# Exidekat/TransformerUpscaler

Measured on AMD Instinct MI355X. Metric: images/sec, FastTransformer 2x 720p->1080p inference, higher is better.
Workload: dtype bf16

## Files before the change

include/tupscale_hip.h:

```cpp
#ifndef TUPSCALE_HIP_H
#define TUPSCALE_HIP_H

#ifdef __cplusplus
extern "C" {
#endif

int tup_abi_version(void);

int tup_conv3x3_c3_fwd(const float* x, const void* wp, const float* bias, const float* in_mask,
                       const void* out_mask, void* out, int B, int H, int W, int relu, void* stream);

int tup_conv3x3_c64_fwd(const void* x, const void* wp, const float* bias, const void* add,
                        const void* mask, void* out, int B, int H, int W, int ntiles, int r,
                        int cout_valid, int relu, int out_mode, int in_r, void* stream);

int tup_decoder_fused_fwd(const void* x, const void* w1, const float* b1, const void* wz, const float* b2,
                          float* seamv, float* cseam, float* out, int B, int H, int W, void* stream);

int tup_conv1_compact_fwd(const float* x, void* xc, int B, int H, int W, void* stream);
int tup_conv12_fused_fwd(const void* xc, const void* w1, const float* b1, const void* w2, const float* b2, void* out,
                         int B, int H, int W, void* stream);

int tup_conv5x5_c64_planar_fwd(const void* x, const void* wp, const float* bias, const void* wv,
                               const float* bv, float* out, int B, int H, int W, int r, int relu, void* stream);

int tup_conv3x3_planar_fwd(const float* x, const float* w28, const float* bias, const float* add,
                           float* out, int B, int H, int W, int r, int clamp01, void* stream);

int tup_resize_aa_fwd(const float* in, float* out, const int* ymin, const int* ysize, const float* yw,
                      int KY, const int* xmin, const int* xsize, const float* xw, int KX, int planes,
                      int Hi, int Wi, int Ho, int Wo, int clamp01, void* stream);

int tup_tail_stream_r2_fwd(const float* x, const float* wfu_t, const float* bfu, const float* wfc_t, const float* bfc,
                           const float* ui, float* out, int B, int H, int W, int clamp01, void* stream);

int tup_tail_stream_r2_resize_fwd(const float* x, const float* wfu_t, const float* bfu, const float* wfc_t, const float* bfc,
                                  const float* ui, float* out, const int* ymin, const int* ysize, const float* yw, int KY,
                                  const int* xmin, const int* xsize, const float* xw, int KX, const int* oxb, const int* oyb,
                                  int B, int H, int W, int Ho, int Wo, int sc, int band_h, int ext, int clamp01, void* stream);

int tup_tail_fused_fwd(const float* x, const float* wfu, const float* bfu, const float* wfc, const float* bfc,
                       const float* ui, float* out, const int* ymin, const int* ysize, const float* yw, int KY,
                       const int* xmin, const int* xsize, const float* xw, int KX, int B, int H, int W, int r,
                       int Ho, int Wo, int EH, int EW, int clamp01, void* stream);

int tup_clamp01_fwd(const float* in, float* out, long long n, void* stream);

int tup_layernorm_fwd(const float* x, const float* gamma, const float* beta, void* y,
                      float* mean, float* rstd, int M, void* stream);

int tup_relpos_bias_expand(const float* table, float* frag, void* stream);

int tup_window_attn_fwd(const void* qkv, const float* bias_frag, void* out, float* lse, int nwin, float drop_p,
                        unsigned int drop_seed, void* stream);

int tup_gemm_tokens_fwd(const void* A, int a_dtype, int lda, const void* Wt, const float* bias,
                        const float* res, const void* aux, void* out, int ldo, int M, int N, int K,
                        int epilogue, float drop_p, unsigned int drop_seed, void* stream);

int tup_ln_gemm_fwd(const float* x, const float* gamma, const float* beta, const void* Wt,
                    const float* bias, void* out, int M, int N, void* stream);

// ... 206 lines not shown
```

transformerupscaler_amd/_lib.py:

```python
from __future__ import annotations

import ctypes
import os
from ctypes import c_double, c_float, c_int, c_longlong, c_uint, c_void_p

_HERE = os.path.dirname(os.path.abspath(__file__))
LIB_PATH = os.environ.get("TUP_LIB_PATH") or os.path.join(_HERE, "libtupscale_hip.so")
ABI_VERSION = 15

P = c_void_p
I = c_int
F = c_float
U = c_uint

SIGNATURES = {
    "tup_abi_version": [],
    "tup_conv3x3_c3_fwd": [P, P, P, P, P, P, I, I, I, I, P],
    "tup_conv3x3_c64_fwd": [P, P, P, P, P, P, I, I, I, I, I, I, I, I, I, P],
    "tup_conv5x5_c64_planar_fwd": [P, P, P, P, P, P, I, I, I, I, I, P],
    "tup_decoder_fused_fwd": [P, P, P, P, P, P, P, P, I, I, I, P],
    "tup_conv1_compact_fwd": [P, P, I, I, I, P],
    "tup_conv12_fused_fwd": [P, P, P, P, P, P, I, I, I, P],
    "tup_conv3x3_planar_fwd": [P, P, P, P, P, I, I, I, I, I, P],
    "tup_resize_aa_fwd": [P, P, P, P, P, I, P, P, P, I, I, I, I, I, I, I, P],
    "tup_tail_fused_fwd": [P, P, P, P, P, P, P, P, P, P, I, P, P, P, I, I, I, I, I, I, I, I, I, I, P],
    "tup_tail_stream_r2_fwd": [P, P, P, P, P, P, P, I, I, I, I, P],
    "tup_tail_stream_r2_resize_fwd": [P] * 7 + [P, P, P, I, P, P, P, I, P, P] + [I] * 9 + [P],
    "tup_clamp01_fwd": [P, P, c_longlong, P],
    "tup_layernorm_fwd": [P, P, P, P, P, P, I, P],
    "tup_relpos_bias_expand": [P, P, P],
    "tup_window_attn_fwd": [P, P, P, P, I, F, U, P],
    "tup_gemm_tokens_fwd": [P, I, I, P, P, P, P, P, I, I, I, I, I, F, U, P],
    "tup_ln_gemm_fwd": [P, P, P, P, P, P, I, I, P],
    "tup_fused_mlp_fwd": [P, P, P, P, P, P, P, I, P],
    "tup_patch_embed_fwd": [P, P, P, P, I, I, I, P],
    "tup_patch_unembed_fwd": [P, I, P, P, P, P, I, I, I, P],
    "tup_rt_patch_embed_fwd": [P, P, P, P, P, I, I, I, P],
    "tup_rt_patch_unembed_fwd": [P, P, P, P, P, I, I, I, P],
    "tup_rt_attention_fwd": [P, P, P, I, I, F, U, P],
    "tup_rt_attention_bwd": [P, P, P, P, P, P, I, I, F, U, P],
    "tup_layernorm128_fwd": [P, P, P, P, P, P, I, P],
    "tup_layernorm128_bwd": [P, P, P, P, P, P, P, P, P, I, P, F, U, P],
    "tup_rt_patch_wgrad": [P, P, P, I, I, I, P],
    "tup_conv3x3_c64_wgrad_s2d": [P, P, P, P, I, I, I, I, I, P],
    "tup_rt_bicubic_bwd": [P] * 10 + [I, I, I, I, I, P],
    "tup_rt_bicubic_bwd_banded": [P] * 7 + [I, P, P, I, P, P, I, I, I, I, I, P, P],
    "tup_relpos_bias_expand_h": [P, P, I, P],
    "tup_relpos_bias_expand_n_h": [P, P, I, P],
    "tup_window_attn_bwd_h": [P, P, P, P, P, P, P, P, I, I, F, U, P],
    "tup_relpos_bias_reduce_h": [P, P, I, P],
# ... 116 lines not shown
```

transformerupscaler_amd/csrc/check_resources.py:

```python
#!/usr/bin/env python3
import json
import os
import re
import subprocess
import sys

GUARDED = [
    ("fused_attn.hip", ["fused_qkv_attn_kernel"]),
    ("block_stream.hip", ["blocks_stream_kernel"]),
    ("fused_blocks.hip", ["fused_mlp_v2_kernel"]),
    ("conv3x3_c64.hip", ["conv_c64_persistent_kernel", "bra_rows_persistent_kernel", "conv3_thin_rows_kernel"]),
    ("conv_thin.hip", ["conv3x3_c3_persistent_kernel"]),
    ("decoder_fused.hip", ["decoder_fused_kernel"]),
    ("conv12_fused.hip", ["conv12_fused_kernel"]),
    ("gemm_tokens.hip", ["gemm_panel2_kernel", "patch_embed_kernel"]),
    ("conv_bwd.hip", ["conv3x3_wgrad_c64_kernel", "conv3x3_wgrad_thin_kernel", "conv3x3_wgrad_c64_det_kernel", "conv3x3_wgrad_thin_det_kernel"]),
    ("branch_a_train.hip", ["bra_wgrad_kernel"]),
    ("gemm_wgrad.hip", ["gemm_wgrad_wide_kernel"]),
    ("gemm_wgrad.hip", ["gemm_wgrad_kernelILi0ELi0ELb1E", "gemm_wgrad_kernelILi0ELi1ELb1E", "gemm_wgrad_kernelILi1ELi0ELb1E",
                        "gemm_wgrad_kernelILi1ELi1ELb1E", "gemm_wgrad_kernelILi1ELi2ELb1E", "colsum_kernelILb0ELb1E", "colsum_kernelILb1ELb1E"]),
    ("attention_bwd.hip", ["layernorm_bwd_kernelILi2ELb1E", "layernorm_bwd_kernelILi3ELb1E"]),
    ("quality_loss.hip", ["quality_loss_bwd_kernel"]),
    ("grad_accumulate.hip", ["grad_accumulate_kernel"]),
    ("step_guard.hip", ["grad_sumsq_kernel", "guard_finish_kernel", "adam_guarded_kernel"]),
    ("patch_pairs.hip", ["patch_pairs_kernel"]),
]
EXEMPT = re.compile(r"fused_qkv_attn_kernel<true, true, true>|fused_qkv_attn_kernelILb1ELb1ELb1E|fused_mlp_v2_kernelILi[1-9]|blocks_stream_kernel<true>|blocks_stream_kernelILb1E")
ALLOWED_BYTES = {"fused_mlp_v2_kernelILi0E": 72}

FIELDS = {
    "sgprs": r"TotalSGPRs: (\d+)", "vgprs": r" VGPRs: (\d+)", "agprs": r"AGPRs: (\d+)",
    "scratch_bytes_per_lane": r"ScratchSize \[bytes/lane\]: (\d+)", "waves_per_simd": r"Occupancy \[waves/SIMD\]: (\d+)",
    "sgpr_spill": r"SGPRs Spill: (\d+)", "vgpr_spill": r"VGPRs Spill: (\d+)",
}


def demangle(names):
    try:
        out = subprocess.run(["c++filt"], input="\n".join(names), capture_output=True, text=True, check=True).stdout.split("\n")
        return dict(zip(names, out))
    except Exception:
        return {n: n for n in names}


def parse(path):
    txt = open(path, errors="replace").read()
    parts = re.split(r"remark: Function Name: (\S+)", txt)
    recs = {}
# ... 58 lines not shown
```

transformerupscaler_amd/csrc/decoder_fused.hip:

```cpp
#include "common.h"

namespace {

constexpr int TH = 8, TW = 32, HALO_W = TW + 2, HALO_H = TH + 2, NPIX_HALO = HALO_H * HALO_W;
constexpr int IN_BYTES = NPIX_HALO * 128, IN_CHUNKS = NPIX_HALO * 8;
constexpr int WROWS = 64, WSLAB = WROWS * 128, WCHUNKS = 9 * WROWS * 8;
constexpr size_t DEC_LDS = (size_t)9 * WSLAB + 2 * (size_t)IN_BYTES + 256;
static_assert(DEC_LDS <= 163840, "LDS budget");

__device__ __attribute__((aligned(16))) unsigned int dec_zero_line[4] = {0u, 0u, 0u, 0u};

#define TUP_ADD_DPP(a, v, ctrl) asm("v_add_f32_dpp %0, %1, %0 " ctrl " row_mask:0xf bank_mask:0xf bound_ctrl:1" : "+v"(a) : "v"(v))

__global__ __launch_bounds__(512, 2) void decoder_fused_kernel(
    const bf16_t* __restrict__ x, const bf16_t* __restrict__ wp, const float* __restrict__ bias,
    const bf16_t* __restrict__ wz, float* __restrict__ part, float* __restrict__ seamv, float* __restrict__ cseam,
    int B, int H, int W, int tilesX, int tilesY)
{
    extern __shared__ __attribute__((aligned(16))) char smem[];
    char* w_lds = smem;
    char* in_lds = smem + 9 * WSLAB;

    const int grp = __builtin_amdgcn_readfirstlane((int)(threadIdx.x >> 8));
    const int tid = threadIdx.x & 255, lane = tid & 63, wave = tid >> 6;
// ... 273 lines not shown
#pragma unroll
        for (int e = 0; e < V; ++e) {
            const int xq = x0 + e;
            float t = bias[c] + v[e];
            if (has_seam) t += sv[e];
            int ctile = -1, side = 0;
            if ((xq & 31) == 31 && xq + 1 < W) { ctile = (xq >> 5) + 1; side = 0; }
            else if ((xq & 31) == 0 && xq > 0) { ctile = (xq >> 5) - 1; side = 1; }
            if (ctile >= 0) {
#pragma unroll
                for (int dy = 0; dy < 3; ++dy) {
                    const int yy = y + dy - 1;
                    if (yy >= 0 && yy < H) t += cseam[((((size_t)b * H + yy) * tilesX + ctile) * 2 + side) * 16 + c * 4 + dy];
                }
            }
            v[e] = t;
        }
        *reinterpret_cast<fv*>(res + o) = v;
    }
}

}

extern "C" int tup_decoder_fused_fwd(const void* x, const void* w1, const float* b1, const void* wz, const float* b2,
                                     float* seamv, float* cseam, float* out, int B, int H, int W, void* stream)
{
    if (B <= 0 || H <= 0 || W <= 0) return 0;
    const int tilesX = (W + TW - 1) / TW, tilesY = (H + TH - 1) / TH;
    const long long nt = (long long)tilesX * tilesY * B;
    if (nt > 0x7fffffffLL || (long long)H * W * 12 > 0x7fffffffLL || (long long)H * tilesX * 128 > 0x7fffffffLL)
        return (int)hipErrorInvalidValue;
    hipStream_t s = reinterpret_cast<hipStream_t>(stream);
    TUP_SET_DYN_LDS(decoder_fused_kernel, DEC_LDS);
    const int grid = (int)(nt < 256 ? nt : 256);
    decoder_fused_kernel<<<dim3(grid), dim3(512), DEC_LDS, s>>>((const bf16_t*)x, (const bf16_t*)w1, b1, (const bf16_t*)wz, out,
                                                                 seamv, cseam, B, H, W, tilesX, tilesY);
    TUP_CHECK_LAUNCH();
    if ((long long)B * H > 0x7fffffffLL) return (int)hipErrorInvalidValue;
    if (W % 4 == 0)
        decoder_finish_kernel<4><<<dim3((unsigned)((W / 4 + 255) / 256), (unsigned)(B * H)), dim3(256), 0, s>>>(out, seamv, cseam, b2, H, W, tilesX);
    else
        decoder_finish_kernel<1><<<dim3((unsigned)((W + 255) / 256), (unsigned)(B * H)), dim3(256), 0, s>>>(out, seamv, cseam, b2, H, W, tilesX);
    TUP_CHECK_LAUNCH();
    return 0;
}
```

transformerupscaler_amd/csrc/tail_stream.hip:

```cpp
#include "common.h"

namespace {

constexpr int TS_COLS = 60;
constexpr int TS_BAND_MIN = 12;

struct TailStreamParams {
    const float* x;
    const float* wfu_t;
    const float* bfu;
    const float* wfc_t;
    const float* bfc;
    const float* ui;
    float* out;
    int B, H, W, nstrip, nband, band_h, clamp01;
    const int* ymin; const int* ysize; const float* yw; int KY;
    const int* xmin; const int* xsize; const float* xw; int KX;
    const int* oxb; const int* oyb;
    int Ho, Wo, sc, ext;
};

TUP_DEVICE float from_left(float v) {
    float r;
    asm volatile("s_nop 1\n\tv_mov_b32_dpp %0, %1 wave_shr:1 row_mask:0xf bank_mask:0xf bound_ctrl:1" : "=v"(r) : "v"(v));
    return r;
}
TUP_DEVICE float from_right(float v) {
    float r;
    asm volatile("s_nop 1\n\tv_mov_b32_dpp %0, %1 wave_shl:1 row_mask:0xf bank_mask:0xf bound_ctrl:1" : "=v"(r) : "v"(v));
    return r;
}

template <bool RESIZE>
__global__ __launch_bounds__(256, 3) void tail_stream_r2_kernel(
    const float* __restrict__ x_arg, const float* __restrict__ wfu_arg, const float* __restrict__ bfu_arg,
    const float* __restrict__ wfc_arg, const float* __restrict__ bfc_arg, const float* __restrict__ ui_arg, float* __restrict__ out_arg,
    const TailStreamParams p)
{
    __shared__ __attribute__((aligned(16))) float wl[36 * 12 + 12 + 4];
    __shared__ __attribute__((aligned(16))) float hb[RESIZE ? 4 : 1][3][128];
    __shared__ __attribute__((aligned(16))) float xwl[RESIZE ? 4 : 1][2][64][4];
    __shared__ __attribute__((aligned(16))) f32x2 vrl[RESIZE ? 4 : 1][6][3][64];
    for (int i = threadIdx.x; i < 27 * 12; i += 256) wl[i] = wfu_arg[i];
    if (threadIdx.x < 27 * 4) wl[324 + threadIdx.x] = wfc_arg[threadIdx.x];
    if (threadIdx.x < 12) wl[432 + threadIdx.x] = bfu_arg[threadIdx.x];
    if (threadIdx.x < 4) wl[444 + threadIdx.x] = threadIdx.x < 3 ? bfc_arg[threadIdx.x] : 0.f;
    __syncthreads();
    const int lane = threadIdx.x & 63;
    const int wid = __builtin_amdgcn_readfirstlane((int)blockIdx.x * 4 + (int)(threadIdx.x >> 6));
    if (wid >= p.B * p.nband * p.nstrip) return;
    const int strip = wid % p.nstrip, band = (wid / p.nstrip) % p.nband, b = wid / (p.nstrip * p.nband);
    const int H = p.H, W = p.W, Hs = 2 * H, Ws = 2 * W;
    const int xcol = strip * (RESIZE ? p.sc : TS_COLS) - 2 + lane;
    const bool colok = xcol >= 0 && xcol < W;
    const bool store_lane = lane >= 2 && lane < 2 + TS_COLS && xcol < W;
    const int y0 = band * p.band_h, y1 = min(y0 + p.band_h, H);
    const int y_end = RESIZE ? min(y1 + p.ext, H) : y1;
    const unsigned xc = colok ? (unsigned)xcol : 0u;
    const __amdgpu_buffer_rsrc_t rx = __builtin_amdgcn_make_buffer_rsrc(const_cast<float*>(x_arg), 0, 0x7fffffff, 0x00020000);
    const __amdgpu_buffer_rsrc_t ru = __builtin_amdgcn_make_buffer_rsrc(const_cast<float*>(ui_arg), 0, 0x7fffffff, 0x00020000);
    const __amdgpu_buffer_rsrc_t ro = __builtin_amdgcn_make_buffer_rsrc(out_arg, 0, 0x7fffffff, 0x00020000);
    const unsigned vx = xc * 4u, vu = xc * 8u;

    float X[3][3];
    float T[3][3][2][2];
    f32x2 xn[3];
    f32x2 un[1][3][2];

    int oxl[2] = {0, 0}, xi[2] = {0, 0};
    bool hval[2] = {false, false};
    int oy = 0, oy_end = 0;
    const int wv = threadIdx.x >> 6;
    if constexpr (RESIZE) {
        const int ox0 = p.oxb[strip], ox1 = p.oxb[strip + 1];
        const int hx0 = 2 * (strip * p.sc - 2);
#pragma unroll
        for (int q = 0; q < 2; ++q) {
            const int ox = ox0 + lane + 64 * q;
            hval[q] = ox < ox1;
            oxl[q] = hval[q] ? ox : ox0;
            xi[q] = hval[q] ? p.xmin[oxl[q]] - hx0 : 4;
            f32x4 wq4;
#pragma unroll
            for (int t = 0; t < 4; ++t) wq4[t] = (hval[q] && t < p.KX) ? p.xw[oxl[q] * p.KX + t] : 0.f;
            *reinterpret_cast<f32x4*>(&xwl[wv][q][lane][0]) = wq4;
        }
        oy = p.oyb[band];
        oy_end = p.oyb[band + 1];
    }
    int nym = 0, nyn = 0;
    float nyw[4] = {0.f, 0.f, 0.f, 0.f};
    auto fetch_row_taps = [&](int row) __attribute__((always_inline)) {
        const int rr = row < oy_end ? row : oy_end - 1;
        nym = p.ymin[rr]; nyn = p.ysize[rr];
#pragma unroll
        for (int a = 0; a < 4; ++a) nyw[a] = a < p.KY ? p.yw[rr * p.KY + a] : 0.f;
    };
    if constexpr (RESIZE) { if (oy < oy_end) fetch_row_taps(oy); }

    auto load_x_row = [&](int row, f32x2 (&dst)[3]) __attribute__((always_inline)) {
        const bool rok = row >= 0 && row < H;
        const int rr = rok ? row : 0;
#pragma unroll
        for (int c = 0; c < 3; ++c)
            dst[c][0] = __builtin_bit_cast(float, __builtin_amdgcn_raw_buffer_load_b32(rx, vx, (((b * 3 + c) * H + rr) * W) * 4, 0));
    };
    auto place_x_row = [&](int row, int slot, const f32x2 (&src)[3]) __attribute__((always_inline)) {
        const bool ok = colok && row >= 0 && row < H;
#pragma unroll
        for (int c = 0; c < 3; ++c) {
            X[slot][c] = ok ? src[c][0] : 0.f;
            asm volatile("" : "+v"(X[slot][c]));
        }
    };
    auto load_ui_rows = [&](int q, int buf) __attribute__((always_inline)) {
        const int qq = (q >= 0 && q < H) ? q : 0;
#pragma unroll
        for (int c = 0; c < 3; ++c)
#pragma unroll
            for (int i = 0; i < 2; ++i)
                un[buf][c][i] = __builtin_bit_cast(f32x2, __builtin_amdgcn_raw_buffer_load_b64(ru, vu, (((b * 3 + c) * Hs + 2 * qq + i) * Ws) * 4, 0));
    };

    const uint32_t wbase = lds_addr(wl);
    f32x4 ring[3][3];
    auto rd = [&](int g) __attribute__((always_inline)) {
#pragma unroll
        for (int j = 0; j < 3; ++j)
            asm volatile("ds_read_b128 %0, %1 offset:%2" : "=v"(ring[g % 3][j]) : "v"(wbase), "i"((g * 12 + j * 4) * 4));
    };
    f32x4 bias[4];
    auto rd_bias = [&]() __attribute__((always_inline)) {
#pragma unroll
        for (int j = 0; j < 3; ++j)
// ... 115 lines not shown
                    *reinterpret_cast<f32x2*>(&hb[wv][c][2 * lane]) = vr[c];
                }
#pragma unroll
                for (int pq = 0; pq < 2; ++pq)
                    if (hval[pq]) {
                        const f32x4 xwt = *reinterpret_cast<const f32x4*>(&xwl[wv][pq][lane][0]);
#pragma unroll
                        for (int c = 0; c < 3; ++c) {
                            float o = xwt[0] * hb[wv][c][xi[pq]];
#pragma unroll
                            for (int t = 1; t < 4; ++t) o = __builtin_fmaf(xwt[t], hb[wv][c][xi[pq] + t], o);
                            if (p.clamp01) o = fminf(fmaxf(o, 0.f), 1.f);
                            __builtin_amdgcn_raw_buffer_store_b32(__builtin_bit_cast(unsigned, o), ro, (unsigned)oxl[pq] * 4u,
                                                                  (((b * 3 + c) * p.Ho + oy) * p.Wo) * 4, 0);
                        }
                    }
                ++oy;
            }
        }
    };

    auto iteration = [&](int r, int S) __attribute__((always_inline)) {
        const int SM = (S + 2) % 3, SP = (S + 1) % 3;
        load_x_row(r + 2, xn);
        stages(r, SM, S, SP, r - 1 >= y0, 0);
        load_ui_rows(r, 0);
        place_x_row(r + 2, SM, xn);
    };

    {
        f32x2 t[3];
        load_x_row(y0 - 2, t); place_x_row(y0 - 2, 1, t);
        load_x_row(y0 - 1, t); place_x_row(y0 - 1, 2, t);
        load_x_row(y0, t);     place_x_row(y0, 0, t);
#pragma unroll
        for (int s = 0; s < 3; ++s)
#pragma unroll
            for (int c = 0; c < 3; ++c)
#pragma unroll
                for (int i = 0; i < 2; ++i)
#pragma unroll
                    for (int e = 0; e < 2; ++e) { T[s][c][i][e] = 0.f; asm volatile("" : "+v"(T[s][c][i][e])); }
    }
    int r = y0 - 1;
    iteration(r, 2); ++r;
    while (r <= y_end) {
        iteration(r, 0); if (++r > y_end) break;
        iteration(r, 1); if (++r > y_end) break;
        iteration(r, 2); ++r;
    }
}

}

namespace {
int launch_tail_stream(TailStreamParams& p, const float* x, const float* wfu_t, const float* bfu, const float* wfc_t, const float* bfc,
                       const float* ui, float* out, bool resize, void* stream)
{
    const long long waves = (long long)p.B * p.nstrip * p.nband;
    if (waves > (1ll << 30) || (long long)p.B * 3 * 4 * p.H * p.W >= (1ll << 29)) return (int)hipErrorInvalidValue;
    const dim3 grid((unsigned)((waves + 3) / 4));
    hipStream_t s = reinterpret_cast<hipStream_t>(stream);
    if (resize) tail_stream_r2_kernel<true><<<grid, dim3(256), 0, s>>>(x, wfu_t, bfu, wfc_t, bfc, ui, out, p);
    else tail_stream_r2_kernel<false><<<grid, dim3(256), 0, s>>>(x, wfu_t, bfu, wfc_t, bfc, ui, out, p);
    TUP_CHECK_LAUNCH();
    return 0;
}
}

extern "C" int tup_tail_stream_r2_fwd(const float* x, const float* wfu_t, const float* bfu, const float* wfc_t, const float* bfc,
                                      const float* ui, float* out, int B, int H, int W, int clamp01, void* stream)
{
    if (B <= 0 || H <= 0 || W <= 0) return 0;
    TailStreamParams p{};
    p.B = B; p.H = H; p.W = W; p.clamp01 = clamp01;
    p.nstrip = (W + TS_COLS - 1) / TS_COLS;
    {
        const long long cols = (long long)B * p.nstrip;
        long long nb = (256 * 4 * 3) / (cols > 0 ? cols : 1);
        if (nb < 1) nb = 1;
        int bh = (int)((H + nb - 1) / nb);
        bh = (bh + 2) / 3 * 3;
        if (bh < TS_BAND_MIN) bh = TS_BAND_MIN;
        p.band_h = bh;
        p.nband = (H + bh - 1) / bh;
    }
    return launch_tail_stream(p, x, wfu_t, bfu, wfc_t, bfc, ui, out, false, stream);
}

extern "C" int tup_tail_stream_r2_resize_fwd(const float* x, const float* wfu_t, const float* bfu, const float* wfc_t, const float* bfc,
                                             const float* ui, float* out, const int* ymin, const int* ysize, const float* yw, int KY,
                                             const int* xmin, const int* xsize, const float* xw, int KX, const int* oxb, const int* oyb,
                                             int B, int H, int W, int Ho, int Wo, int sc, int band_h, int ext, int clamp01, void* stream)
{
    if (B <= 0 || H <= 0 || W <= 0) return 0;
    if (sc < 1 || sc > TS_COLS || band_h < 3 || band_h % 3 != 0 || ext < 0 || ext > 2 || Ho < 1 || Wo < 1 || KX < 1 || KY < 1)
        return (int)hipErrorInvalidValue;
    if ((long long)B * 3 * Ho * Wo >= (1ll << 29)) return (int)hipErrorInvalidValue;
    TailStreamParams p{};
    p.B = B; p.H = H; p.W = W; p.clamp01 = clamp01;
    p.nstrip = (W + sc - 1) / sc;
    p.band_h = band_h;
    p.nband = (H + band_h - 1) / band_h;
    p.ymin = ymin; p.ysize = ysize; p.yw = yw; p.KY = KY; p.xmin = xmin; p.xsize = xsize; p.xw = xw; p.KX = KX;
    p.oxb = oxb; p.oyb = oyb; p.Ho = Ho; p.Wo = Wo; p.sc = sc; p.ext = ext;
    return launch_tail_stream(p, x, wfu_t, bfu, wfc_t, bfc, ui, out, true, stream);
}
```

transformerupscaler_amd/engine.py:

```python
from __future__ import annotations

import os

import math
from typing import Dict, Optional, Tuple

import torch

from . import ops
from .weights import BLOCKS, VALID_SCALES, upsampler_layout


stage_timer = None
fuse_attention = 3


class _NullCtx:
    def __enter__(self):
        return None

    def __exit__(self, *a):
        return False


def _stage(name: str):
    return stage_timer(name) if stage_timer is not None else _NullCtx()


def resolve_scale(h: int, w: int, res_out, upscale_factor: Optional[int]):
    if upscale_factor is not None:
        res_out = (h * upscale_factor, w * upscale_factor)
    else:
        upscale_factor = math.ceil(max(res_out[0] / h, res_out[1] / w))
    if upscale_factor not in VALID_SCALES:
        raise ValueError(f"Requested scale={upscale_factor} was not built.")
    return (int(res_out[0]), int(res_out[1])), int(upscale_factor)


blocks_in_one_launch = True
stream_blocks = True
STREAM_MIN_WINDOWS = 512
stream_bf16_tokens = True
fuse_blocks = True
fuse_tail = True
stream_tail = True
fuse_decoder = True
fuse_conv12 = True


def _block_operands(pk, i, bias_frags):
    return (pk[f"b{i}.qkv.whn"], pk[f"b{i}.qkv.bhn"], bias_frags[i], pk[f"b{i}.proj.wpp"], pk[f"b{i}.proj.b"],
            pk[f"b{i}.fc1.wfqn"], pk[f"b{i}.fc1.bqn"], pk[f"b{i}.fc2.wh4"], pk[f"b{i}.fc2.b"])


def transformer_blocks(pk: Dict[str, torch.Tensor], x: torch.Tensor, bias_frags, capture=None, bf16_out: bool = False):
    if (fuse_blocks and fuse_attention >= 3 and capture is None and "b0.stream.0" in pk and blocks_in_one_launch and stream_blocks
            and x.shape[0] // 64 >= STREAM_MIN_WINDOWS):
        table = ops.stream_table([tuple(pk[f"b{i}.stream.{j}"] for j in range(7)) for i in range(BLOCKS)])
        return ops.blocks_stream(x, table, out_bf16=bf16_out and stream_bf16_tokens)
    if fuse_blocks and fuse_attention >= 3 and capture is None and "b0.proj.wpp" in pk and blocks_in_one_launch:
        table = ops.block_table([_block_operands(pk, i, bias_frags) for i in range(BLOCKS)])
        return ops.fused_blocks32(x, table)
    for i in range(BLOCKS):
        qkv = None
        if fuse_blocks and fuse_attention >= 3 and capture is None and f"b{i}.proj.wpp" in pk:
            ops.fused_block(x, *_block_operands(pk, i, bias_frags))
            continue
        if fuse_blocks and fuse_attention == 2 and capture is None and f"b{i}.proj.wpp" in pk:
            ops.fused_attn_block(x, pk[f"b{i}.norm1.w"], pk[f"b{i}.norm1.b"], pk[f"b{i}.qkv.wh"], pk[f"b{i}.qkv.bh"], bias_frags[i],
                                 pk[f"b{i}.proj.wpp"], pk[f"b{i}.proj.b"])
# ... 46 lines not shown
    if fuse_branch_a and "bra.w" in pk:
        for si, (_, r) in enumerate(stages[:-1]):
            up = ops.conv_c64(up, pk[f"up1.{si}.w"], pk[f"up1.{si}.b"], r, relu=False)
        with _stage("branch_a"):
            upscaled_input = ops.branch_a_composed(up, pk["bra.w"], pk["bra.b"], pk["bra.wv"], pk["bra.bv"], stages[-1][1])
    else:
        for si, (_, r) in enumerate(stages):
            with _stage(f"up1.{si}"):
                up = ops.conv_c64(up, pk[f"up1.{si}.w"], pk[f"up1.{si}.b"], r, relu=False)
        upscaled_input = ops.conv_c64_thin(up, pk["up1_conv.w"], None, 3, relu=True)
        if cap is not None:
            cap["up1"] = up
    if cap is not None:
        cap["feat"] = feat; cap["upscaled_input"] = upscaled_input
    del up
    with _stage("patch_embed"):
        xw = ops.patch_embed(feat, pk["pe.w"], pk["pe.b"])
    if cap is not None:
        cap["win_in"] = xw.clone()
    with _stage("blocks"):
        xw = transformer_blocks(pk, xw, bias_frags, cap, bf16_out=cap is None)
    with _stage("unembed"):
        combined = ops.patch_unembed(xw, pk["pu.w"], pk["pu.b"], feat)
    if fuse_decoder and fuse_tail and cap is None and "dec2.wz" in pk:
        with _stage("decoder"):
            residual = ops.decoder_fused(combined, pk["dec1.w"], pk["dec1.b"], pk["dec2.wz"], pk["dec2.b"])
    else:
        with _stage("dec1"):
            dec = ops.conv_c64(combined, pk["dec1.w"], pk["dec1.b"], 1, relu=True)
        with _stage("dec2"):
            residual = ops.conv_c64_thin(dec, pk["dec2.w"], pk["dec2.b"], 3, relu=False)
    if cap is not None:
        cap["combined"] = combined; cap["dec"] = dec; cap["residual"] = residual
    t = residual
    hs, ws = H * scale, W * scale
    needs_resize = bool(require_ratio) and tuple(res_out) != (hs, hs) and tuple(res_out) != (hs, ws)
    fu = upsampler_layout(scale)
    if fuse_tail and cap is None:
        for si, (_, r) in enumerate(fu[:-1]):
            t = ops.conv_planar(t, pk[f"fu.{si}.w"], pk[f"fu.{si}.b"], r)
        li = len(fu) - 1
        if (stream_tail and fu[li][1] == 2 and "tail.wfu_t" in pk
                and ops.tail_stream_fits(t.shape[0], t.shape[2], t.shape[3], tuple(res_out) if needs_resize else None)):
            with _stage("tail"):
                out = ops.tail_stream_r2(t, pk["tail.wfu_t"], pk[f"fu.{li}.b"], pk["tail.wfc_t"], pk["fuc.b"], upscaled_input,
                                         clamp=True, out_hw=tuple(res_out) if needs_resize else None)
                if out is None:
                    out = ops.tail_stream_r2(t, pk["tail.wfu_t"], pk[f"fu.{li}.b"], pk["tail.wfc_t"], pk["fuc.b"], upscaled_input, clamp=False)
                    out = ops.resize_aa(out, tuple(res_out), clamp=True)
            return out
        with _stage("tail"):
            out = ops.tail_fused(t, pk[f"fu.{li}.w"], pk[f"fu.{li}.b"], pk["fuc.w"], pk["fuc.b"], upscaled_input, fu[li][1],
                                 tuple(res_out) if needs_resize else (hs, ws), clamp=True)
        return out
    for si, (_, r) in enumerate(fu):
        t = ops.conv_planar(t, pk[f"fu.{si}.w"], pk[f"fu.{si}.b"], r)
    out = ops.conv_planar(t, pk["fuc.w"], pk["fuc.b"], 1, add=upscaled_input, clamp=not needs_resize)
    if cap is not None:
        cap["sum"] = out
    if needs_resize:
        out = ops.resize_aa(out, res_out, clamp=True)
    return out
```

transformerupscaler_amd/ops.py:

```python
from __future__ import annotations

import contextlib
import os
import struct

import numpy as np
import torch

from . import _lib
from .resize_taps import aa_taps

BF16, F32 = torch.bfloat16, torch.float32


_raw_stream = getattr(torch._C, "_cuda_getCurrentRawStream", None)
_cur_dev = torch.cuda.current_device


def _stream():
    if _raw_stream is not None:
        return _raw_stream(_cur_dev())
    return torch.cuda.current_stream().cuda_stream


# ... 77 lines not shown
    nt = r * r
    if out is None:
        out = torch.empty((B, H * r, W * r, 64), dtype=BF16, device=x.device)
    else:
        _chk(out, BF16, (B, H * r, W * r, 64), "out")
    _lib.call("tup_conv3x3_c64_fwd", _chk(x, BF16, None, "x"), _chk(wp, BF16, (nt, in_r * in_r, 9, 64, 64), "wp"),
              _opt(bias, F32, (nt, 64), "bias"), _opt(add, BF16, out.shape, "add"), _opt(mask, BF16, out.shape, "mask"),
              out.data_ptr(), B, H, W, nt, r, 64, int(relu), 0, in_r, _stream())
    return out


def conv_c64_thin(x, wp, bias, cout, relu=False, out=None):
    B, H, W, C = x.shape
    assert C == 64 and 1 <= cout <= 16
    if out is None:
        out = torch.empty((B, cout, H, W), dtype=F32, device=x.device)
    else:
        _chk(out, F32, (B, cout, H, W), "out")
    _lib.call("tup_conv3x3_c64_fwd", _chk(x, BF16, None, "x"), _chk(wp, BF16, (1, 1, 9, 16, 64), "wp"),
              _opt(bias, F32, (cout,), "bias"), None, None, out.data_ptr(), B, H, W, 1, 1, cout, int(relu), 1, 1, _stream())
    return out


def decoder_fused(x, w1, b1, wz, b2):
    B, H, W, C = x.shape
    assert C == 64
    out = torch.empty((B, 3, H, W), dtype=F32, device=x.device)
    seamv = torch.empty((B, 3, H, W), dtype=F32, device=x.device)
    cseam = torch.empty((B, H, (W + 31) // 32, 32), dtype=F32, device=x.device)
    _lib.call("tup_decoder_fused_fwd", _chk(x, BF16, None, "x"), _chk(w1, BF16, (1, 1, 9, 64, 64), "w1"), _chk(b1, F32, (1, 64), "b1"),
              _chk(wz, BF16, (48, 64), "wz"), _chk(b2, F32, (3,), "b2"), seamv.data_ptr(), cseam.data_ptr(), out.data_ptr(),
              B, H, W, _stream())
    return out


def branch_a_composed(x, wp, bias, wv, bv, r, relu=True):
    B, H, W, C = x.shape
    assert C == 64 and r in (2, 3, 6)
    rows, n = {2: 16, 3: 32, 6: 112}[r], 3 * r * r
    out = torch.empty((B, 3, H * r, W * r), dtype=F32, device=x.device)
    _lib.call("tup_conv5x5_c64_planar_fwd", _chk(x, BF16, None, "x"), _chk(wp, BF16, (1, 1, 25, rows, 64), "wp"),
              _chk(bias, F32, (n,), "bias"), _chk(wv, BF16, (9, n, 25, 64), "wv"), _chk(bv, F32, (9, n), "bv"),
              out.data_ptr(), B, H, W, r, int(relu), _stream())
    return out


def conv_planar(x, w28, bias, r=1, add=None, clamp=False):
    B, C, H, W = x.shape
    assert C == 3
    cout = 3 * r * r
    both = clamp == "both"
    shape = (B, 3, H * r, W * r)
# ... 78 lines not shown
            for s_ in range(nstrip):
                a, b_ = int(oxb[s_]), int(oxb[s_ + 1])
                if b_ > a:
                    ok &= bool((xlo[a:b_] + xn[a:b_]).max() <= 2 * s_ * sc + 120) and b_ - a <= 128
            for k_ in range(nband):
                a, b_ = int(oyb[k_]), int(oyb[k_ + 1])
                if b_ > a:
                    ok &= bool((ylo[a:b_] + yn[a:b_]).max() <= 2 * min(H, (k_ + 1) * bh + ext))
            if ok:
                t = lambda arr: torch.from_numpy(np.ascontiguousarray(arr)).to(device)
                plan = (t(ylo), t(yn), t(yw), ky, t(xlo), t(xn), t(xw), kx, t(oxb), t(oyb), sc, bh, ext)
        _TAP_CACHE[key] = plan
    return _TAP_CACHE[key]


def tail_stream_fits(B, H, W, out_hw=None):
    if B * 12 * H * W >= 1 << 29:
        return False
    if out_hw is not None and tuple(out_hw) != (2 * H, 2 * W) and B * 3 * int(out_hw[0]) * int(out_hw[1]) >= 1 << 29:
        return False
    return True


def tail_stream_r2(x, wfu_t, bfu, wfc_t, bfc, ui, clamp=True, out_hw=None):
    B, C, H, W = x.shape
    args = (_chk(x, F32, (B, 3, H, W), "x"), _chk(wfu_t, F32, (27, 12), "wfu_t"), _chk(bfu, F32, (12,), "bfu"),
            _chk(wfc_t, F32, (27, 4), "wfc_t"), _chk(bfc, F32, (3,), "bfc"), _chk(ui, F32, (B, 3, 2 * H, 2 * W), "ui"))
    if out_hw is None or tuple(out_hw) == (2 * H, 2 * W):
        out = torch.empty((B, 3, 2 * H, 2 * W), dtype=F32, device=x.device)
        _lib.call("tup_tail_stream_r2_fwd", *args, out.data_ptr(), B, H, W, int(clamp), _stream())
        return out
    Ho, Wo = int(out_hw[0]), int(out_hw[1])
    plan = _tail_stream_plan(x.device, B, H, W, Ho, Wo)
    if plan is None:
        return None
    ylo, yn, yw, ky, xlo, xn, xw, kx, oxb, oyb, sc, bh, ext = plan
    out = torch.empty((B, 3, Ho, Wo), dtype=F32, device=x.device)
    _lib.call("tup_tail_stream_r2_resize_fwd", *args, out.data_ptr(), ylo.data_ptr(), yn.data_ptr(), yw.data_ptr(), ky,
              xlo.data_ptr(), xn.data_ptr(), xw.data_ptr(), kx, oxb.data_ptr(), oyb.data_ptr(), B, H, W, Ho, Wo, sc, bh, ext,
              int(clamp), _stream())
    return out


def clamp01(x):
    out = torch.empty_like(x)
    _lib.call("tup_clamp01_fwd", _chk(x, F32, None, "x"), out.data_ptr(), x.numel(), _stream())
    return out


def layernorm(x, gamma, beta, save_stats=False):
    M, D = x.shape
    assert D == 192
    y = torch.empty((M, 192), dtype=BF16, device=x.device)
    mean = rstd = None
    if save_stats:
        mean = torch.empty((M,), dtype=F32, device=x.device)
        rstd = torch.empty((M,), dtype=F32, device=x.device)
    _lib.call("tup_layernorm_fwd", _chk(x, F32, None, "x"), _chk(gamma, F32, (192,), "gamma"),
              _chk(beta, F32, (192,), "beta"), y.data_ptr(), None if mean is None else mean.data_ptr(),
              None if rstd is None else rstd.data_ptr(), M, _stream())
    return (y, mean, rstd) if save_stats else y
# ... 1009 lines not shown
```

Before: 2638.

## Fuse decoder finish pass into streaming tail kernel

Skips the separate decoder_finish kernel and passes the decoder's partial output, vertical seam sums and column-seam buffers straight to the streaming r2 tail kernel. The tail adds bias, seam and column-seam contributions while loading each input row. This removes one kernel launch and a full read-modify-write of the 3-channel residual. In exchange the tail kernel issues extra seamv and cseam loads per row and uses more registers.

New measurement: 2719 (median of 6 runs). +3.1%, better.

```diff
diff --git a/include/tupscale_hip.h b/include/tupscale_hip.h
--- a/include/tupscale_hip.h
+++ b/include/tupscale_hip.h
@@ -16,6 +16,9 @@
 
 int tup_decoder_fused_fwd(const void* x, const void* w1, const float* b1, const void* wz, const float* b2,
                           float* seamv, float* cseam, float* out, int B, int H, int W, void* stream);
+
+int tup_decoder_fused_parts_fwd(const void* x, const void* w1, const float* b1, const void* wz,
+                                float* part, float* seamv, float* cseam, int B, int H, int W, void* stream);
 
 int tup_conv1_compact_fwd(const float* x, void* xc, int B, int H, int W, void* stream);
 int tup_conv12_fused_fwd(const void* xc, const void* w1, const float* b1, const void* w2, const float* b2, void* out,
@@ -38,6 +41,15 @@
                                   const float* ui, float* out, const int* ymin, const int* ysize, const float* yw, int KY,
                                   const int* xmin, const int* xsize, const float* xw, int KX, const int* oxb, const int* oyb,
                                   int B, int H, int W, int Ho, int Wo, int sc, int band_h, int ext, int clamp01, void* stream);
+
+int tup_tail_stream_r2_parts_fwd(const float* part, const float* seamv, const float* cseam, const float* b2, int tilesX,
+                                 const float* wfu_t, const float* bfu, const float* wfc_t, const float* bfc,
+                                 const float* ui, float* out, int B, int H, int W, int clamp01, void* stream);
+int tup_tail_stream_r2_resize_parts_fwd(const float* part, const float* seamv, const float* cseam, const float* b2, int tilesX,
+                                        const float* wfu_t, const float* bfu, const float* wfc_t, const float* bfc,
+                                        const float* ui, float* out, const int* ymin, const int* ysize, const float* yw, int KY,
+                                        const int* xmin, const int* xsize, const float* xw, int KX, const int* oxb, const int* oyb,
+                                        int B, int H, int W, int Ho, int Wo, int sc, int band_h, int ext, int clamp01, void* stream);
 
 int tup_tail_fused_fwd(const float* x, const float* wfu, const float* bfu, const float* wfc, const float* bfc,
                        const float* ui, float* out, const int* ymin, const int* ysize, const float* yw, int KY,
diff --git a/transformerupscaler_amd/_lib.py b/transformerupscaler_amd/_lib.py
--- a/transformerupscaler_amd/_lib.py
+++ b/transformerupscaler_amd/_lib.py
@@ -19,6 +19,7 @@
     "tup_conv3x3_c64_fwd": [P, P, P, P, P, P, I, I, I, I, I, I, I, I, I, P],
     "tup_conv5x5_c64_planar_fwd": [P, P, P, P, P, P, I, I, I, I, I, P],
     "tup_decoder_fused_fwd": [P, P, P, P, P, P, P, P, I, I, I, P],
+    "tup_decoder_fused_parts_fwd": [P, P, P, P, P, P, P, I, I, I, P],
     "tup_conv1_compact_fwd": [P, P, I, I, I, P],
     "tup_conv12_fused_fwd": [P, P, P, P, P, P, I, I, I, P],
     "tup_conv3x3_planar_fwd": [P, P, P, P, P, I, I, I, I, I, P],
@@ -26,6 +27,8 @@
     "tup_tail_fused_fwd": [P, P, P, P, P, P, P, P, P, P, I, P, P, P, I, I, I, I, I, I, I, I, I, I, P],
     "tup_tail_stream_r2_fwd": [P, P, P, P, P, P, P, I, I, I, I, P],
     "tup_tail_stream_r2_resize_fwd": [P] * 7 + [P, P, P, I, P, P, P, I, P, P] + [I] * 9 + [P],
+    "tup_tail_stream_r2_parts_fwd": [P, P, P, P, I] + [P] * 6 + [I, I, I, I, P],
+    "tup_tail_stream_r2_resize_parts_fwd": [P, P, P, P, I] + [P] * 6 + [P, P, P, I, P, P, P, I, P, P] + [I] * 9 + [P],
     "tup_clamp01_fwd": [P, P, c_longlong, P],
     "tup_layernorm_fwd": [P, P, P, P, P, P, I, P],
     "tup_relpos_bias_expand": [P, P, P],
diff --git a/transformerupscaler_amd/csrc/check_resources.py b/transformerupscaler_amd/csrc/check_resources.py
--- a/transformerupscaler_amd/csrc/check_resources.py
+++ b/transformerupscaler_amd/csrc/check_resources.py
@@ -24,6 +24,7 @@
     ("grad_accumulate.hip", ["grad_accumulate_kernel"]),
     ("step_guard.hip", ["grad_sumsq_kernel", "guard_finish_kernel", "adam_guarded_kernel"]),
     ("patch_pairs.hip", ["patch_pairs_kernel"]),
+    ("tail_stream.hip", ["tail_stream_r2_kernel"]),
 ]
 EXEMPT = re.compile(r"fused_qkv_attn_kernel<true, true, true>|fused_qkv_attn_kernelILb1ELb1ELb1E|fused_mlp_v2_kernelILi[1-9]|blocks_stream_kernel<true>|blocks_stream_kernelILb1E")
 ALLOWED_BYTES = {"fused_mlp_v2_kernelILi0E": 72}
diff --git a/transformerupscaler_amd/csrc/decoder_fused.hip b/transformerupscaler_amd/csrc/decoder_fused.hip
--- a/transformerupscaler_amd/csrc/decoder_fused.hip
+++ b/transformerupscaler_amd/csrc/decoder_fused.hip
@@ -319,10 +319,10 @@
 
 }
 
-extern "C" int tup_decoder_fused_fwd(const void* x, const void* w1, const float* b1, const void* wz, const float* b2,
-                                     float* seamv, float* cseam, float* out, int B, int H, int W, void* stream)
-{
-    if (B <= 0 || H <= 0 || W <= 0) return 0;
+namespace {
+int launch_decoder_parts(const void* x, const void* w1, const float* b1, const void* wz, float* part, float* seamv, float* cseam,
+                         int B, int H, int W, void* stream)
+{
     const int tilesX = (W + TW - 1) / TW, tilesY = (H + TH - 1) / TH;
     const long long nt = (long long)tilesX * tilesY * B;
     if (nt > 0x7fffffffLL || (long long)H * W * 12 > 0x7fffffffLL || (long long)H * tilesX * 128 > 0x7fffffffLL)
@@ -330,9 +330,20 @@
     hipStream_t s = reinterpret_cast<hipStream_t>(stream);
     TUP_SET_DYN_LDS(decoder_fused_kernel, DEC_LDS);
     const int grid = (int)(nt < 256 ? nt : 256);
-    decoder_fused_kernel<<<dim3(grid), dim3(512), DEC_LDS, s>>>((const bf16_t*)x, (const bf16_t*)w1, b1, (const bf16_t*)wz, out,
+    decoder_fused_kernel<<<dim3(grid), dim3(512), DEC_LDS, s>>>((const bf16_t*)x, (const bf16_t*)w1, b1, (const bf16_t*)wz, part,
                                                                  seamv, cseam, B, H, W, tilesX, tilesY);
     TUP_CHECK_LAUNCH();
+    return 0;
+}
+}
+
+extern "C" int tup_decoder_fused_fwd(const void* x, const void* w1, const float* b1, const void* wz, const float* b2,
+                                     float* seamv, float* cseam, float* out, int B, int H, int W, void* stream)
+{
+    if (B <= 0 || H <= 0 || W <= 0) return 0;
+    const int tilesX = (W + TW - 1) / TW;
+    if (const int err = launch_decoder_parts(x, w1, b1, wz, out, seamv, cseam, B, H, W, stream)) return err;
+    hipStream_t s = reinterpret_cast<hipStream_t>(stream);
     if ((long long)B * H > 0x7fffffffLL) return (int)hipErrorInvalidValue;
     if (W % 4 == 0)
         decoder_finish_kernel<4><<<dim3((unsigned)((W / 4 + 255) / 256), (unsigned)(B * H)), dim3(256), 0, s>>>(out, seamv, cseam, b2, H, W, tilesX);
@@ -341,3 +352,10 @@
     TUP_CHECK_LAUNCH();
     return 0;
 }
+
+extern "C" int tup_decoder_fused_parts_fwd(const void* x, const void* w1, const float* b1, const void* wz,
+                                           float* part, float* seamv, float* cseam, int B, int H, int W, void* stream)
+{
+    if (B <= 0 || H <= 0 || W <= 0) return 0;
+    return launch_decoder_parts(x, w1, b1, wz, part, seamv, cseam, B, H, W, stream);
+}
diff --git a/transformerupscaler_amd/csrc/tail_stream.hip b/transformerupscaler_amd/csrc/tail_stream.hip
--- a/transformerupscaler_amd/csrc/tail_stream.hip
+++ b/transformerupscaler_amd/csrc/tail_stream.hip
@@ -18,6 +18,8 @@
     const int* xmin; const int* xsize; const float* xw; int KX;
     const int* oxb; const int* oyb;
     int Ho, Wo, sc, ext;
+    const float* seamv; const float* cseam; const float* b2;
+    int tilesX;
 };
 
 TUP_DEVICE float from_left(float v) {
@@ -31,7 +33,7 @@
     return r;
 }
 
-template <bool RESIZE>
+template <bool RESIZE, bool PARTS>
 __global__ __launch_bounds__(256, 3) void tail_stream_r2_kernel(
     const float* __restrict__ x_arg, const float* __restrict__ wfu_arg, const float* __restrict__ bfu_arg,
     const float* __restrict__ wfc_arg, const float* __restrict__ bfc_arg, const float* __restrict__ ui_arg, float* __restrict__ out_arg,
@@ -61,10 +63,26 @@
     const __amdgpu_buffer_rsrc_t ru = __builtin_amdgcn_make_buffer_rsrc(const_cast<float*>(ui_arg), 0, 0x7fffffff, 0x00020000);
     const __amdgpu_buffer_rsrc_t ro = __builtin_amdgcn_make_buffer_rsrc(out_arg, 0, 0x7fffffff, 0x00020000);
     const unsigned vx = xc * 4u, vu = xc * 8u;
+    __amdgpu_buffer_rsrc_t rsv = rx, rcs = rx;
+    unsigned vcs = 0u;
+    bool edge = false;
+    float b2v[3] = {0.f, 0.f, 0.f};
+    if constexpr (PARTS) {
+        rsv = __builtin_amdgcn_make_buffer_rsrc(const_cast<float*>(p.seamv), 0, 0x7fffffff, 0x00020000);
+        rcs = __builtin_amdgcn_make_buffer_rsrc(const_cast<float*>(p.cseam), 0, 0x7fffffff, 0x00020000);
+        int ctile = -1, side = 0;
+        if ((xcol & 31) == 31 && xcol + 1 < W) ctile = (xcol >> 5) + 1;
+        else if ((xcol & 31) == 0 && xcol > 0) { ctile = (xcol >> 5) - 1; side = 1; }
+        edge = colok && ctile >= 0;
+        vcs = edge ? (unsigned)(ctile * 2 + side) * 64u : 0u;
+#pragma unroll
+        for (int c = 0; c < 3; ++c) b2v[c] = p.b2[c];
+    }
 
     float X[3][3];
     float T[3][3][2][2];
     f32x2 xn[3];
+    float cn[3][3];
     f32x2 un[1][3][2];
 
     int oxl[2] = {0, 0}, xi[2] = {0, 0};
@@ -98,18 +116,43 @@
     };
     if constexpr (RESIZE) { if (oy < oy_end) fetch_row_taps(oy); }
 
-    auto load_x_row = [&](int row, f32x2 (&dst)[3]) __attribute__((always_inline)) {
+    auto load_x_row = [&](int row, f32x2 (&dst)[3], float (&cd)[3][3]) __attribute__((always_inline)) {
         const bool rok = row >= 0 && row < H;
         const int rr = rok ? row : 0;
 #pragma unroll
-        for (int c = 0; c < 3; ++c)
+        for (int c = 0; c < 3; ++c) {
             dst[c][0] = __builtin_bit_cast(float, __builtin_amdgcn_raw_buffer_load_b32(rx, vx, (((b * 3 + c) * H + rr) * W) * 4, 0));
-    };
-    auto place_x_row = [&](int row, int slot, const f32x2 (&src)[3]) __attribute__((always_inline)) {
+            if constexpr (PARTS)
+                dst[c][1] = __builtin_bit_cast(float, __builtin_amdgcn_raw_buffer_load_b32(rsv, vx, (((b * 3 + c) * H + rr) * W) * 4, 0));
+        }
+        if constexpr (PARTS) {
+#pragma unroll
+            for (int dy = 0; dy < 3; ++dy) {
+                const int yy = min(max(row + dy - 1, 0), H - 1);
+#pragma unroll
+                for (int c = 0; c < 3; ++c)
+                    cd[c][dy] = __builtin_bit_cast(float, __builtin_amdgcn_raw_buffer_load_b32(
+                        rcs, vcs, ((b * H + yy) * p.tilesX * 32 + c * 4 + dy) * 4, 0));
+            }
+        }
+    };
+    auto place_x_row = [&](int row, int slot, const f32x2 (&src)[3], const float (&cd)[3][3]) __attribute__((always_inline)) {
         const bool ok = colok && row >= 0 && row < H;
+        const int ys = (row & 1) ? row + 1 : row - 1;
+        const bool has_seam = ys >= 0 && ys < H;
 #pragma unroll
         for (int c = 0; c < 3; ++c) {
-            X[slot][c] = ok ? src[c][0] : 0.f;
+            float t = src[c][0];
+            if constexpr (PARTS) {
+                t = b2v[c] + t;
+                t = has_seam ? t + src[c][1] : t;
+#pragma unroll
+                for (int dy = 0; dy < 3; ++dy) {
+                    const bool cok = edge && row + dy - 1 >= 0 && row + dy - 1 < H;
+                    t = cok ? t + cd[c][dy] : t;
+                }
+            }
+            X[slot][c] = ok ? t : 0.f;
             asm volatile("" : "+v"(X[slot][c]));
         }
     };
@@ -271,17 +314,18 @@
 
     auto iteration = [&](int r, int S) __attribute__((always_inline)) {
         const int SM = (S + 2) % 3, SP = (S + 1) % 3;
-        load_x_row(r + 2, xn);
+        load_x_row(r + 2, xn, cn);
         stages(r, SM, S, SP, r - 1 >= y0, 0);
         load_ui_rows(r, 0);
-        place_x_row(r + 2, SM, xn);
+        place_x_row(r + 2, SM, xn, cn);
     };
 
     {
         f32x2 t[3];
-        load_x_row(y0 - 2, t); place_x_row(y0 - 2, 1, t);
-        load_x_row(y0 - 1, t); place_x_row(y0 - 1, 2, t);
-        load_x_row(y0, t);     place_x_row(y0, 0, t);
+        float tc[3][3];
+        load_x_row(y0 - 2, t, tc); place_x_row(y0 - 2, 1, t, tc);
+        load_x_row(y0 - 1, t, tc); place_x_row(y0 - 1, 2, t, tc);
+        load_x_row(y0, t, tc);     place_x_row(y0, 0, t, tc);
 #pragma unroll
         for (int s = 0; s < 3; ++s)
 #pragma unroll
@@ -303,22 +347,30 @@
 }
 
 namespace {
-int launch_tail_stream(TailStreamParams& p, const float* x, const float* wfu_t, const float* bfu, const float* wfc_t, const float* bfc,
-                       const float* ui, float* out, bool resize, void* stream)
+struct TailParts { const float* part; const float* seamv; const float* cseam; const float* b2; int tilesX; };
+
+int launch_tail_stream(TailStreamParams& p, const float* x, const TailParts* parts, const float* wfu_t, const float* bfu,
+                       const float* wfc_t, const float* bfc, const float* ui, float* out, bool resize, void* stream)
 {
     const long long waves = (long long)p.B * p.nstrip * p.nband;
     if (waves > (1ll << 30) || (long long)p.B * 3 * 4 * p.H * p.W >= (1ll << 29)) return (int)hipErrorInvalidValue;
+    if (parts) {
+        if (parts->tilesX != (p.W + 31) / 32 || (long long)p.B * p.H * parts->tilesX * 32 >= (1ll << 29)) return (int)hipErrorInvalidValue;
+        x = parts->part;
+        p.seamv = parts->seamv; p.cseam = parts->cseam; p.b2 = parts->b2; p.tilesX = parts->tilesX;
+    }
     const dim3 grid((unsigned)((waves + 3) / 4));
     hipStream_t s = reinterpret_cast<hipStream_t>(stream);
-    if (resize) tail_stream_r2_kernel<true><<<grid, dim3(256), 0, s>>>(x, wfu_t, bfu, wfc_t, bfc, ui, out, p);
-    else tail_stream_r2_kernel<false><<<grid, dim3(256), 0, s>>>(x, wfu_t, bfu, wfc_t, bfc, ui, out, p);
+    if (resize && parts) tail_stream_r2_kernel<true, true><<<grid, dim3(256), 0, s>>>(x, wfu_t, bfu, wfc_t, bfc, ui, out, p);
+    else if (resize) tail_stream_r2_kernel<true, false><<<grid, dim3(256), 0, s>>>(x, wfu_t, bfu, wfc_t, bfc, ui, out, p);
+    else if (parts) tail_stream_r2_kernel<false, true><<<grid, dim3(256), 0, s>>>(x, wfu_t, bfu, wfc_t, bfc, ui, out, p);
+    else tail_stream_r2_kernel<false, false><<<grid, dim3(256), 0, s>>>(x, wfu_t, bfu, wfc_t, bfc, ui, out, p);
     TUP_CHECK_LAUNCH();
     return 0;
 }
-}
-
-extern "C" int tup_tail_stream_r2_fwd(const float* x, const float* wfu_t, const float* bfu, const float* wfc_t, const float* bfc,
-                                      const float* ui, float* out, int B, int H, int W, int clamp01, void* stream)
+
+int tail_stream_plain(const float* x, const TailParts* parts, const float* wfu_t, const float* bfu, const float* wfc_t, const float* bfc,
+                      const float* ui, float* out, int B, int H, int W, int clamp01, void* stream)
 {
     if (B <= 0 || H <= 0 || W <= 0) return 0;
     TailStreamParams p{};
@@ -334,13 +386,13 @@
         p.band_h = bh;
         p.nband = (H + bh - 1) / bh;
     }
-    return launch_tail_stream(p, x, wfu_t, bfu, wfc_t, bfc, ui, out, false, stream);
-}
-
-extern "C" int tup_tail_stream_r2_resize_fwd(const float* x, const float* wfu_t, const float* bfu, const float* wfc_t, const float* bfc,
-                                             const float* ui, float* out, const int* ymin, const int* ysize, const float* yw, int KY,
-                                             const int* xmin, const int* xsize, const float* xw, int KX, const int* oxb, const int* oyb,
-                                             int B, int H, int W, int Ho, int Wo, int sc, int band_h, int ext, int clamp01, void* stream)
+    return launch_tail_stream(p, x, parts, wfu_t, bfu, wfc_t, bfc, ui, out, false, stream);
+}
+
+int tail_stream_resize(const float* x, const TailParts* parts, const float* wfu_t, const float* bfu, const float* wfc_t, const float* bfc,
+                       const float* ui, float* out, const int* ymin, const int* ysize, const float* yw, int KY,
+                       const int* xmin, const int* xsize, const float* xw, int KX, const int* oxb, const int* oyb,
+                       int B, int H, int W, int Ho, int Wo, int sc, int band_h, int ext, int clamp01, void* stream)
 {
     if (B <= 0 || H <= 0 || W <= 0) return 0;
     if (sc < 1 || sc > TS_COLS || band_h < 3 || band_h % 3 != 0 || ext < 0 || ext > 2 || Ho < 1 || Wo < 1 || KX < 1 || KY < 1)
@@ -353,5 +405,41 @@
     p.nband = (H + band_h - 1) / band_h;
     p.ymin = ymin; p.ysize = ysize; p.yw = yw; p.KY = KY; p.xmin = xmin; p.xsize = xsize; p.xw = xw; p.KX = KX;
     p.oxb = oxb; p.oyb = oyb; p.Ho = Ho; p.Wo = Wo; p.sc = sc; p.ext = ext;
-    return launch_tail_stream(p, x, wfu_t, bfu, wfc_t, bfc, ui, out, true, stream);
-}
+    return launch_tail_stream(p, x, parts, wfu_t, bfu, wfc_t, bfc, ui, out, true, stream);
+}
+}
+
+extern "C" int tup_tail_stream_r2_fwd(const float* x, const float* wfu_t, const float* bfu, const float* wfc_t, const float* bfc,
+                                      const float* ui, float* out, int B, int H, int W, int clamp01, void* stream)
+{
+    return tail_stream_plain(x, nullptr, wfu_t, bfu, wfc_t, bfc, ui, out, B, H, W, clamp01, stream);
+}
+
+extern "C" int tup_tail_stream_r2_resize_fwd(const float* x, const float* wfu_t, const float* bfu, const float* wfc_t, const float* bfc,
+                                             const float* ui, float* out, const int* ymin, const int* ysize, const float* yw, int KY,
+                                             const int* xmin, const int* xsize, const float* xw, int KX, const int* oxb, const int* oyb,
+                                             int B, int H, int W, int Ho, int Wo, int sc, int band_h, int ext, int clamp01, void* stream)
+{
+    return tail_stream_resize(x, nullptr, wfu_t, bfu, wfc_t, bfc, ui, out, ymin, ysize, yw, KY, xmin, xsize, xw, KX, oxb, oyb,
+                              B, H, W, Ho, Wo, sc, band_h, ext, clamp01, stream);
+}
+
+extern "C" int tup_tail_stream_r2_parts_fwd(const float* part, const float* seamv, const float* cseam, const float* b2, int tilesX,
+                                            const float* wfu_t, const float* bfu, const float* wfc_t, const float* bfc,
+                                            const float* ui, float* out, int B, int H, int W, int clamp01, void* stream)
+{
+    const TailParts parts{part, seamv, cseam, b2, tilesX};
+    return tail_stream_plain(nullptr, &parts, wfu_t, bfu, wfc_t, bfc, ui, out, B, H, W, clamp01, stream);
+}
+
+extern "C" int tup_tail_stream_r2_resize_parts_fwd(const float* part, const float* seamv, const float* cseam, const float* b2, int tilesX,
+                                                   const float* wfu_t, const float* bfu, const float* wfc_t, const float* bfc,
+                                                   const float* ui, float* out, const int* ymin, const int* ysize, const float* yw, int KY,
+                                                   const int* xmin, const int* xsize, const float* xw, int KX, const int* oxb,
+                                                   const int* oyb, int B, int H, int W, int Ho, int Wo, int sc, int band_h, int ext,
+                                                   int clamp01, void* stream)
+{
+    const TailParts parts{part, seamv, cseam, b2, tilesX};
+    return tail_stream_resize(nullptr, &parts, wfu_t, bfu, wfc_t, bfc, ui, out, ymin, ysize, yw, KY, xmin, xsize, xw, KX, oxb, oyb,
+                              B, H, W, Ho, Wo, sc, band_h, ext, clamp01, stream);
+}
diff --git a/transformerupscaler_amd/engine.py b/transformerupscaler_amd/engine.py
--- a/transformerupscaler_amd/engine.py
+++ b/transformerupscaler_amd/engine.py
@@ -46,6 +46,7 @@
 stream_tail = True
 fuse_decoder = True
 fuse_conv12 = True
+fuse_decoder_finish = True
 
 
 def _block_operands(pk, i, bias_frags):
@@ -138,9 +139,18 @@
         xw = transformer_blocks(pk, xw, bias_frags, cap, bf16_out=cap is None)
     with _stage("unembed"):
         combined = ops.patch_unembed(xw, pk["pu.w"], pk["pu.b"], feat)
+    hs, ws = H * scale, W * scale
+    needs_resize = bool(require_ratio) and tuple(res_out) != (hs, hs) and tuple(res_out) != (hs, ws)
+    fu = upsampler_layout(scale)
+    tail_out_hw = tuple(res_out) if needs_resize else None
+    parts = None
     if fuse_decoder and fuse_tail and cap is None and "dec2.wz" in pk:
+        unfinished = (fuse_decoder_finish and stream_tail and len(fu) == 1 and fu[0][1] == 2 and "tail.wfu_t" in pk
+                      and ops.tail_stream_fits(B, H, W, tail_out_hw))
         with _stage("decoder"):
-            residual = ops.decoder_fused(combined, pk["dec1.w"], pk["dec1.b"], pk["dec2.wz"], pk["dec2.b"])
+            residual = ops.decoder_fused(combined, pk["dec1.w"], pk["dec1.b"], pk["dec2.wz"], pk["dec2.b"], finish=not unfinished)
+        if unfinished:
+            parts, residual = residual, residual[0]
     else:
         with _stage("dec1"):
             dec = ops.conv_c64(combined, pk["dec1.w"], pk["dec1.b"], 1, relu=True)
@@ -149,22 +159,21 @@
     if cap is not None:
         cap["combined"] = combined; cap["dec"] = dec; cap["residual"] = residual
     t = residual
-    hs, ws = H * scale, W * scale
-    needs_resize = bool(require_ratio) and tuple(res_out) != (hs, hs) and tuple(res_out) != (hs, ws)
-    fu = upsampler_layout(scale)
     if fuse_tail and cap is None:
         for si, (_, r) in enumerate(fu[:-1]):
             t = ops.conv_planar(t, pk[f"fu.{si}.w"], pk[f"fu.{si}.b"], r)
         li = len(fu) - 1
         if (stream_tail and fu[li][1] == 2 and "tail.wfu_t" in pk
-                and ops.tail_stream_fits(t.shape[0], t.shape[2], t.shape[3], tuple(res_out) if needs_resize else None)):
+                and ops.tail_stream_fits(t.shape[0], t.shape[2], t.shape[3], tail_out_hw)):
             with _stage("tail"):
                 out = ops.tail_stream_r2(t, pk["tail.wfu_t"], pk[f"fu.{li}.b"], pk["tail.wfc_t"], pk["fuc.b"], upscaled_input,
-                                         clamp=True, out_hw=tuple(res_out) if needs_resize else None)
+                                         clamp=True, out_hw=tail_out_hw, parts=parts)
                 if out is None:
-                    out = ops.tail_stream_r2(t, pk["tail.wfu_t"], pk[f"fu.{li}.b"], pk["tail.wfc_t"], pk["fuc.b"], upscaled_input, clamp=False)
+                    out = ops.tail_stream_r2(t, pk["tail.wfu_t"], pk[f"fu.{li}.b"], pk["tail.wfc_t"], pk["fuc.b"], upscaled_input,
+                                             clamp=False, parts=parts)
                     out = ops.resize_aa(out, tuple(res_out), clamp=True)
             return out
+        assert parts is None
         with _stage("tail"):
             out = ops.tail_fused(t, pk[f"fu.{li}.w"], pk[f"fu.{li}.b"], pk["fuc.w"], pk["fuc.b"], upscaled_input, fu[li][1],
                                  tuple(res_out) if needs_resize else (hs, ws), clamp=True)
diff --git a/transformerupscaler_amd/ops.py b/transformerupscaler_amd/ops.py
--- a/transformerupscaler_amd/ops.py
+++ b/transformerupscaler_amd/ops.py
@@ -123,12 +123,18 @@
     return out
 
 
-def decoder_fused(x, w1, b1, wz, b2):
+def decoder_fused(x, w1, b1, wz, b2, finish=True):
     B, H, W, C = x.shape
     assert C == 64
     out = torch.empty((B, 3, H, W), dtype=F32, device=x.device)
     seamv = torch.empty((B, 3, H, W), dtype=F32, device=x.device)
     cseam = torch.empty((B, H, (W + 31) // 32, 32), dtype=F32, device=x.device)
+    if not finish:
+        _chk(b2, F32, (3,), "b2")
+        _lib.call("tup_decoder_fused_parts_fwd", _chk(x, BF16, None, "x"), _chk(w1, BF16, (1, 1, 9, 64, 64), "w1"),
+                  _chk(b1, F32, (1, 64), "b1"), _chk(wz, BF16, (48, 64), "wz"), out.data_ptr(), seamv.data_ptr(), cseam.data_ptr(),
+                  B, H, W, _stream())
+        return out, seamv, cseam, b2
     _lib.call("tup_decoder_fused_fwd", _chk(x, BF16, None, "x"), _chk(w1, BF16, (1, 1, 9, 64, 64), "w1"), _chk(b1, F32, (1, 64), "b1"),
               _chk(wz, BF16, (48, 64), "wz"), _chk(b2, F32, (3,), "b2"), seamv.data_ptr(), cseam.data_ptr(), out.data_ptr(),
               B, H, W, _stream())
@@ -253,21 +259,32 @@
     return True
 
 
-def tail_stream_r2(x, wfu_t, bfu, wfc_t, bfc, ui, clamp=True, out_hw=None):
-    B, C, H, W = x.shape
-    args = (_chk(x, F32, (B, 3, H, W), "x"), _chk(wfu_t, F32, (27, 12), "wfu_t"), _chk(bfu, F32, (12,), "bfu"),
-            _chk(wfc_t, F32, (27, 4), "wfc_t"), _chk(bfc, F32, (3,), "bfc"), _chk(ui, F32, (B, 3, 2 * H, 2 * W), "ui"))
+def tail_stream_r2(x, wfu_t, bfu, wfc_t, bfc, ui, clamp=True, out_hw=None, parts=None):
+    if parts is not None:
+        part, seamv, cseam, b2 = parts
+        B, C, H, W = part.shape
+        dev, tiles_x = part.device, (W + 31) // 32
+        head = (_chk(part, F32, (B, 3, H, W), "part"), _chk(seamv, F32, (B, 3, H, W), "seamv"),
+                _chk(cseam, F32, (B, H, tiles_x, 32), "cseam"), _chk(b2, F32, (3,), "b2"), tiles_x)
+        suffix = "_parts_fwd"
+    else:
+        B, C, H, W = x.shape
+        dev = x.device
+        head = (_chk(x, F32, (B, 3, H, W), "x"),)
+        suffix = "_fwd"
+    args = head + (_chk(wfu_t, F32, (27, 12), "wfu_t"), _chk(bfu, F32, (12,), "bfu"),
+                   _chk(wfc_t, F32, (27, 4), "wfc_t"), _chk(bfc, F32, (3,), "bfc"), _chk(ui, F32, (B, 3, 2 * H, 2 * W), "ui"))
     if out_hw is None or tuple(out_hw) == (2 * H, 2 * W):
-        out = torch.empty((B, 3, 2 * H, 2 * W), dtype=F32, device=x.device)
-        _lib.call("tup_tail_stream_r2_fwd", *args, out.data_ptr(), B, H, W, int(clamp), _stream())
+        out = torch.empty((B, 3, 2 * H, 2 * W), dtype=F32, device=dev)
+        _lib.call("tup_tail_stream_r2" + suffix, *args, out.data_ptr(), B, H, W, int(clamp), _stream())
         return out
     Ho, Wo = int(out_hw[0]), int(out_hw[1])
-    plan = _tail_stream_plan(x.device, B, H, W, Ho, Wo)
+    plan = _tail_stream_plan(dev, B, H, W, Ho, Wo)
     if plan is None:
         return None
     ylo, yn, yw, ky, xlo, xn, xw, kx, oxb, oyb, sc, bh, ext = plan
-    out = torch.empty((B, 3, Ho, Wo), dtype=F32, device=x.device)
-    _lib.call("tup_tail_stream_r2_resize_fwd", *args, out.data_ptr(), ylo.data_ptr(), yn.data_ptr(), yw.data_ptr(), ky,
+    out = torch.empty((B, 3, Ho, Wo), dtype=F32, device=dev)
+    _lib.call("tup_tail_stream_r2_resize" + suffix, *args, out.data_ptr(), ylo.data_ptr(), yn.data_ptr(), yw.data_ptr(), ky,
               xlo.data_ptr(), xn.data_ptr(), xw.data_ptr(), kx, oxb.data_ptr(), oyb.data_ptr(), B, H, W, Ho, Wo, sc, bh, ext,
               int(clamp), _stream())
     return out
```
